# SyamVangara/multigrid-petsc

Hardware: AMD Instinct MI355X
Metric: fp64 DOF-updates/sec per V-cycle at 1024^3 (higher is better)
Workload: dtype f64

## Files before the change

include/mgk.h:

```cpp
#ifndef MGK_H
#define MGK_H
#include <stddef.h>
#ifdef __cplusplus
extern "C" {
#endif

#define MGK_XOFF 16
#define MGK_EINVAL  10001
#define MGK_ENOGPU  10002
#define MGK_ECOMM   10003

typedef struct mgk_ctx mgk_ctx;

typedef struct mgk_geom {
    int  dim;
    int  nx, ny, nz;
    int  pitch;
    long plane;
    long org;
    long total;
} mgk_geom;

int  mgk_geom_init(mgk_geom *g, int dim, int nx, int ny, int nz);

// ... 351 lines not shown
    MGK_TUNE_J2_RING_OLD       = 39,
    MGK_TUNE_SRR_TY2           = 40,
    MGK_TUNE_SRR_TY4           = 41,
    MGK_TUNE_J2_ZERO_RINGB     = 45,
    MGK_TUNE_PJ2_COPY          = 46,
    MGK_TUNE_J3_2D_MARCH       = 50,
    MGK_TUNE_J3_2D_CHUNK4      = 51,
    MGK_TUNE_J3_2D_CHUNK8      = 52,
    MGK_TUNE_DISPATCH_ORDER    = 53,
    MGK_TUNE_XCD_ORDER         = 54,
    MGK_TUNE_RR2D_MARCH        = 55,
    MGK_TUNE_RR2D_SHORT        = 56,
    MGK_TUNE_RESERVED_57       = 57,
    MGK_TUNE_J3_2D_ODD_DOWN    = 58,
    MGK_TUNE_J3_2D_ALL_DOWN    = 59,
    MGK_TUNE_J3_2D_STORE_PLAIN = 60,
    MGK_TUNE_J3_2D_STORE_NT    = 61,
    MGK_TUNE_J3_3D_TY2         = 62,
    MGK_TUNE_J3_3D_TY3         = 63,
    MGK_TUNE_J3_3D_ROWWISE     = 64,
    MGK_TUNE_NO_EXACT_FMA      = 65,
    MGK_TUNE_J3_3D_WAVES       = 66,
    MGK_TUNE_J3_3D_STACKED     = 67,
    MGK_TUNE_J3_3D_STACKED_DISPATCH = 68
};

void mgk_set_tuning(int variant, int zchunk);

#ifdef __cplusplus
}
#endif
#endif
```

include/mgk_sweep3.h:

```cpp
#ifndef MGK_SWEEP3_H
#define MGK_SWEEP3_H
#include "mgk.h"
#ifdef __cplusplus
extern "C" {
#endif

int  mgk_jacobi3_mid_ok_f64(const mgk_geom *g);
int  mgk_jacobi3_sumsq_mid_f64(mgk_ctx *ctx, const mgk_geom *g, const double *coef, double dinv, double scale,
                               const double *b, const double *u, double *unew, double *sumsq_host, void *stream);

#ifdef __cplusplus
}
#endif
#endif
```

include/mgsolve.h:

```cpp
#ifndef MGSOLVE_H
#define MGSOLVE_H
#include "mgk.h"
#ifdef __cplusplus
extern "C" {
#endif

typedef enum { MG_KSP_RICHARDSON = 0, MG_KSP_CHEBYSHEV = 1 } mg_ksp_type;
typedef enum { MG_PREC_FP64 = 0, MG_PREC_MIXED = 1 } mg_precision;
typedef enum { MG_PC_JACOBI = 0, MG_PC_LINE_Y = 1, MG_PC_LINE_X = 2, MG_PC_LINE_ALT = 3, MG_PC_RBGS = 4 } mg_pc_type;

typedef enum mg_fuse_bits {
    MG_FUSE_RESNORM = 1,
    MG_FUSE_PROLONG_SWEEP = 2,
    MG_FUSE_RES_RESTRICT = 4,
    MG_FUSE_NORM_SWEEP = 8,
    MG_FUSE_MIXED_CORRECT = 16,
    MG_FUSE_PAIRS = 32,
    MG_FUSE_RES_RESTRICT_SMALL = 128,
    MG_FUSE_COARSE_ZERO_SWEEP = 256,
    MG_FUSE_LDS_TAIL = 512,
    MG_FUSE_SWEEP_RESTRICT = 1024,
    MG_FUSE_ZERO_TRIPLE = 2048,
    MG_FUSE_PROLONG_PAIR = 4096,
    MG_FUSE_TRIPLE_2D = 8192,
// ... 39 lines not shown
struct mg_comm;

int  mg_solver_create(mg_solver **s, const mg_config *cfg, struct mg_comm *comm);
void mg_solver_destroy(mg_solver *s);
const char *mg_last_error(void);

int  mg_solver_set_rhs_problem(mg_solver *s);
int  mg_solver_set_rhs_host(mg_solver *s, const double *b_compact);
int  mg_solver_reset(mg_solver *s);
int  mg_solver_solve(mg_solver *s);
int  mg_solver_cycles(mg_solver *s, int ncycles);
int  mg_solver_fmg(mg_solver *s, int nu);
int  mg_solver_solve_fmg(mg_solver *s, int nu);
int  mg_solver_solve_gmres(mg_solver *s, int restart);
int  mg_solver_sync(mg_solver *s);

int    mg_solver_iterations(const mg_solver *s);
double mg_solver_bnorm(const mg_solver *s);
const double *mg_solver_rnorm(const mg_solver *s);
double mg_solver_solve_seconds(const mg_solver *s);

int  mg_solver_num_levels(const mg_solver *s);
int  mg_solver_tail_level(const mg_solver *s);
int  mg_solver_level_n(const mg_solver *s, int level);
int  mg_solver_level_local_planes(const mg_solver *s, int level, int *z0);
long mg_solver_local_unknowns(const mg_solver *s);
double mg_solver_dof_updates_per_cycle(const mg_solver *s);

int  mg_solver_get_solution(mg_solver *s, double *u_compact);
int  mg_solver_error_norms(mg_solver *s, double err[3]);

int  mg_solver_profile(mg_solver *s, int enable);
int  mg_solver_profile_read(mg_solver *s, double *total_ms, int *launches);
int  mg_solver_profile_read_kind(mg_solver *s, int kind, double *total_ms, int *launches);

void mg_get_ranges(int totaln, int procs, int *ranges);
int  mg_grid_n(int npts, int grid);
long mg_grid_to_global(int dim, int n, int k, int i, int j);
void mg_global_to_grid(int dim, int n, long idx, int *k, int *i, int *j);
int  mg_slab_range(int npts, int levels_dist, int level, int rank, int nranks, int *z0, int *z1);

#ifdef __cplusplus
}
#endif
#endif
```

multigrid_petsc_amd/csrc/mg_solver.c:

```c
#include "mgsolve.h"
#include "mg_comm.h"
#include "mg_solver_internal.h"
#include <math.h>
#include <stdio.h>
#include <stdlib.h>
#include <string.h>
#include <time.h>

#define MG_PI 3.14159265358979323846
static __thread char g_mgerr[512] = "ok";
const char *mg_last_error(void) { return g_mgerr; }
static int mgfail(int code, const char *what) {
    snprintf(g_mgerr, sizeof(g_mgerr), "%s (code %d; kernel layer: %s)", what, code, mgk_last_error());
    return code;
}

typedef struct mg_ops {
    int esz;
    int (*jacobi_range)(mgk_ctx *, const mgk_geom *, const double *, double, double, const void *, const void *, void *, int, int, void *);
    int (*jacobi_zero)(mgk_ctx *, const mgk_geom *, double, double, const void *, void *, void *);
    int (*residual)(mgk_ctx *, const mgk_geom *, const double *, const void *, const void *, void *, void *);
    int (*restrict_fw)(mgk_ctx *, const mgk_geom *, const mgk_geom *, const void *, void *, void *);
    int (*prolong_add)(mgk_ctx *, const mgk_geom *, const mgk_geom *, const void *, void *, void *);
    int (*prolong_jacobi)(mgk_ctx *, const mgk_geom *, const mgk_geom *, const double *, double, double, const void *, const void *, const void *, void *, void *);
// ... 935 lines not shown
    }
    F->u_ghost_ok = 0;
    return 0;
}

static int pjp_ok(const mg_solver *s, int P) {
    const mg_level *L = &s->L[0];
    const int need = MG_FUSE_PROLONG_PAIR | MG_FUSE_SWEEP_RESTRICT | MG_FUSE_PAIRS | MG_FUSE_NORM_SWEEP | MG_FUSE_PROLONG_SWEEP | MG_FUSE_RESNORM;
    if ((s->cfg.fuse & need) != need || P != 0 || s->cfg.dim != 3 || s->cfg.mesh || s->cfg.ksp_type != MG_KSP_RICHARDSON) return 0;
    if (s->cfg.v[0] != 3 || s->levels < 2 || s->lgraph == 1 || L->n < s->cfg.pair_min_n || s->last_cycle) return 0;
    if (L->distributed) {
        const mg_level *Lc = &s->L[1];
        const int hi = s->cfg.rank < s->cfg.nranks - 1;
        if (!(s->cfg.fuse & MG_FUSE_PROLONG_PAIR_SLAB) || !Lc->distributed || !L->f[0].far || !Lc->f[0].far || L->nz_min < 8 || Lc->nz_min < 4) return 0;
        return mgk_prolong_jacobi2_slab_ok_f64(&L->f[0].g, &Lc->f[0].g, hi) && mgk_jacobi2_sumsq_ok_f64(&L->f[0].g);
    }
    return mgk_prolong_jacobi2_ok_f64(&L->f[0].g, &s->L[1].f[0].g) && mgk_jacobi2_sumsq_ok_f64(&L->f[0].g);
}
static int triple_mid_ok(const mg_solver *s) {
    if (!(s->cfg.fuse & MG_FUSE_TRIPLE_MID) || !mg_triple_mid_pass || !mg_triple_mid_fits) return 0;
    if (s->cfg.nranks != 1 || s->L[0].distributed || s->cfg.v[0] != 3 || s->lgraph == 1) return 0;
    return srr_ok(s, 0, 0) && mg_triple_mid_fits(s);
}
static int finalize_iterate(mg_solver *s) {
    if (!s->iterate_behind) return 0;
    mg_level *L = &s->L[0];
    mg_fset *F = &L->f[0];
    if (L->distributed) {
        CHK(ensure_u_ghosts(s, 0, L));
        CHK(mgk_jacobi_range_f64(s->ctx, &F->g, L->coef, L->dinv, s->cfg.scale, (const double *)F->b, (const double *)F->u, (double *)F->tmp, 0, F->g.nz, NULL));
    } else
    CHK(mgk_jacobi_f64(s->ctx, &F->g, L->coef, L->dinv, s->cfg.scale, (const double *)F->b, (const double *)F->u, (double *)F->tmp, NULL));
    swap_ptr(&F->u, &F->tmp);
    mgi_u_rewritten(F);
    s->iterate_behind = 0; s->spec_valid = 0;
    return 0;
}

static int prolong_smooth(mg_solver *s, int P, int l) {
    mg_level *Lf = &s->L[l], *Lc = &s->L[l + 1];
    mg_fset *F = &Lf->f[P], *Cq = &Lc->f[P];
    const mg_ops *O = &OPS[P];
    const int v0 = s->cfg.v[0];
    if (!(s->cfg.fuse & MG_FUSE_PROLONG_SWEEP) || (s->cfg.ksp_type != MG_KSP_RICHARDSON && !j3_2d_ok(s, P, l, v0)) || v0 < 1) {
        CHK(prolong_from(s, P, l));
        return smooth(s, P, l, v0, 0);
// ... 31 lines not shown
        CHK(mgk_stream_wait(s->ctx, cs, ms));
        Cq->u_ghost_pending = 0; Cq->u_ghost_ok = 1;
        F->u_ghost_pending = 0; F->u_ghost_ok = 1; F->b_ghost_ok = 1;
        if (split) {
            if (lo) CHK(PJ2S(0, 4));
            if (hi) CHK(PJ2S(nz - 2, nz));
        } else CHK(PJ2S(0, nz));
#undef PJ2S
        swap_ptr(&F->u, &F->tmp);
        mgi_u_rewritten(F);
        s->sweep_owed = 1;
        return 0;
    }
    if (l == 0 && pjp_ok(s, P)) {
        void *t = triple_mid_ok(s) ? prof_begin_kind(s, 0, 1) : NULL;
        int rc2 = mgk_prolong_jacobi2_f64(s->ctx, &F->g, &Cq->g, Lf->coef, Lf->dinv, s->cfg.scale, (const double *)F->b, (const double *)Cq->u,
                                          (const double *)F->u, (double *)F->tmp, NULL);
        prof_end(s, t);
        CHK(rc2);
        swap_ptr(&F->u, &F->tmp);
        mgi_u_rewritten(F);
        s->sweep_owed = 1;
        return 0;
    }
    mgk_geom gc = Cq->g;
    const void *ucoarse = Cq->u;
    if (Lf->distributed && !Lc->distributed) {
        int c0 = s->zstart[s->cfg.rank], c1 = s->zstart[s->cfg.rank + 1];
        gc.nz = c1 - c0;
        ucoarse = (const char *)Cq->u + (size_t)O->esz * (size_t)c0 * (size_t)Cq->g.plane;
    } else if (Lc->distributed) {
        CHK(begin_u_ghosts(s, P, Lc));
    }
    if (Lf->distributed && s->cfg.overlap && Lf->nz_min >= 4 && s->cfg.dim == 3) {
        const int nz = F->g.nz;
        CHK(begin_u_ghosts(s, P, Lf));
        CHK(O->prolong_jacobi_range(s->ctx, &F->g, &gc, Lf->coef, Lf->dinv, s->cfg.scale, F->b, ucoarse, F->u, F->tmp, 2, nz - 1, NULL));
        if (Lc->distributed) CHK(ensure_u_ghosts(s, P, Lc));
        CHK(ensure_u_ghosts(s, P, Lf));
        CHK(O->prolong_jacobi_range(s->ctx, &F->g, &gc, Lf->coef, Lf->dinv, s->cfg.scale, F->b, ucoarse, F->u, F->tmp, 0, 2, NULL));
        CHK(O->prolong_jacobi_range(s->ctx, &F->g, &gc, Lf->coef, Lf->dinv, s->cfg.scale, F->b, ucoarse, F->u, F->tmp, nz - 1, nz, NULL));
    } else {
        if (Lf->distributed && Lc->distributed) CHK(ensure_u_ghosts(s, P, Lc));
        CHK(ensure_u_ghosts(s, P, Lf));
        if (s->cfg.mesh) CHK(mgk_prolong_jacobi_rowcoef_f64(s->ctx, &F->g, &gc, Lf->ctab, Lf->dtab, s->cfg.scale, (const double *)F->b,
                                                            (const double *)ucoarse, (const double *)F->u, (double *)F->tmp, NULL));
// ... 464 lines not shown
    if (!rc) rc = finalize_iterate(s);
    if (rc) return rc;
    double *ss = (double *)malloc(sizeof(double) * (size_t)(ncycles > 0 ? ncycles : 1));
    if (!ss) return mgfail(MGK_EINVAL, "mg_solver_cycles: out of host memory");
    rc = reduce_slots(s, s->d_norms, ncycles, ss);
    if (rc) { free(ss); return mgfail(rc, "mg_solver_cycles: reading the deferred norms"); }
    for (int q = 0; q < ncycles; q++) s->rnorm[it0 + 1 + q] = sqrt(ss[q]);
    if (ncycles > 0) s->rchk = s->rnorm[it0 + ncycles];
    free(ss);
    return 0;
}

int mg_solver_sync(mg_solver *s) {
    CHK(mgk_sync(s->ctx, NULL));
    if (s->comm && s->comm->check) { int rcc = s->comm->check(s->comm); if (rcc) return mgfail(rcc, mg_comm_last_error()); }
    return 0;
}
int mg_solver_iterations(const mg_solver *s) { return s->iter; }
double mg_solver_bnorm(const mg_solver *s) { return s->bnorm; }
const double *mg_solver_rnorm(const mg_solver *s) { return s->rnorm; }
double mg_solver_solve_seconds(const mg_solver *s) { return s->solve_seconds; }
int mg_solver_num_levels(const mg_solver *s) { return s->levels; }
int mg_solver_tail_level(const mg_solver *s) { return s ? s->ltail : 0; }
int mg_solver_level_n(const mg_solver *s, int l) { return (l >= 0 && l < s->levels) ? s->L[l].n : -1; }
int mg_solver_level_local_planes(const mg_solver *s, int l, int *z0) {
    if (l < 0 || l >= s->levels) return -1;
    if (z0) *z0 = s->L[l].z0;
    return s->L[l].nzl;
}
long mg_solver_local_unknowns(const mg_solver *s) {
    const mgk_geom *g = &s->L[0].f[0].g;
    return (long)g->nx * g->ny * g->nz;
}
double mg_solver_dof_updates_per_cycle(const mg_solver *s) {
    double tot = 0.0;
    for (int l = 0; l < s->levels; l++) {
        double N = pow((double)s->L[l].n, (double)s->cfg.dim);
        int sweeps = (l == s->levels - 1 && s->levels > 1) ? s->cfg.v[1] : 2 * s->cfg.v[0];
        if (s->levels == 1) sweeps = s->cfg.v[0];
        tot += sweeps * N;
    }
    return tot;
}

int mgi_fail(int code, const char *what) { return mgfail(code, what); }
int mgi_upload(mg_solver *s, const double *h, size_t n, double **d) { return upload(s, h, n, d); }
// ... 30 lines not shown
```

multigrid_petsc_amd/csrc/mg_solver_internal.h:

```cpp
#ifndef MG_SOLVER_INTERNAL_H
#define MG_SOLVER_INTERNAL_H
#include "mgsolve.h"
#include "mg_comm.h"
#include "mg_cheby_coefs.h"

#define MG_MAX_LEVELS 32
#define MG_MAX_TIMERS 4096

#define MG_FUSE_POINT_JACOBI_PASSES (MG_FUSE_PROLONG_SWEEP | MG_FUSE_NORM_SWEEP | MG_FUSE_PAIRS | MG_FUSE_COARSE_ZERO_SWEEP | MG_FUSE_LDS_TAIL | \
                                     MG_FUSE_SWEEP_RESTRICT | MG_FUSE_ZERO_TRIPLE | MG_FUSE_PROLONG_PAIR | MG_FUSE_TRIPLE_2D | \
                                     MG_FUSE_PROLONG_PAIR_SLAB | MG_FUSE_CHEBY | MG_FUSE_TRIPLE_MID)
#define MG_FUSE_NO_ROW_TABLE_FORM   (MG_FUSE_MIXED_CORRECT | MG_FUSE_RES_RESTRICT_SMALL)

typedef struct mg_fset {
    mgk_geom g;
    void *u, *b, *rv, *tmp;
    int guess_nonzero;
    int u_ghost_ok;
    int u_ghost_pending;
    int jz_ready;
    int last_sweep_pending;
    int b_ghost_ok;
    int pre_done;
    void *far;
// ... 24 lines not shown
    mgk_ctx *ctx;
    mg_comm *comm;
    int levels, ldist;
    mg_level L[MG_MAX_LEVELS];
    int *zstart;
    double *rnorm;
    int rnorm_cap;
    int iter;
    double bnorm, rchk;
    int started;
    int deferring;
    double *d_norms; int d_norms_cap;
    double *pin; int pin_cap;
    int spec_valid;
    int sweep_owed;
    int last_cycle;
    int iterate_behind;
    double solve_seconds;
    int lgraph;
    int ltail;
    void *coarse_graph[2];
    void *graph_u[2], *graph_tmp[2];
    int graph_rerecorded;
    int prof_on, prof_n;
    void *timers[MG_MAX_TIMERS];
    unsigned char timer_kind[MG_MAX_TIMERS];
    int prof_kind;
    int ntimers_created;
    void *gm_field[MGK_KRYLOV_MAX + 3];
    int gm_nfields, gm_restart;
    double *gm_hdev;
};

enum { MG_CHEBY_ZERO = 0, MG_CHEBY_PLAIN = 1, MG_CHEBY_PROLONG = 2, MG_CHEBY_NORM = 3 };
extern int mg_cheby_pass(mg_solver *s, int l, int kind, double *sumsq) __attribute__((weak));
extern int mg_cheby_tail(mg_solver *s) __attribute__((weak));

extern int mg_line_tables(mg_solver *s, int l, const double *ctab_host) __attribute__((weak));
extern int mg_line_smooth(mg_solver *s, int l, int maxit) __attribute__((weak));
extern int mg_xline_tables(mg_solver *s, int l, const double *ctab_host) __attribute__((weak));
extern int mg_xline_smooth(mg_solver *s, int l, int maxit) __attribute__((weak));
extern int mg_line_chunk_tables(mg_solver *s, int l, const double *ctab_host) __attribute__((weak));
extern int mg_line_chunk_smooth(mg_solver *s, int l, int maxit) __attribute__((weak));
extern int mg_xline_chunk_tables(mg_solver *s, int l, const double *ctab_host) __attribute__((weak));
extern int mg_xline_chunk_smooth(mg_solver *s, int l, int maxit) __attribute__((weak));
extern int mg_line_tail(mg_solver *s) __attribute__((weak));
extern int mg_rbgs_smooth(mg_solver *s, int l, int maxit) __attribute__((weak));
extern int mg_rbgs_prolong_smooth(mg_solver *s, int l, int maxit) __attribute__((weak));
extern int mg_triple_mid_fits(const mg_solver *s) __attribute__((weak));
extern int mg_triple_mid_pass(mg_solver *s, double *sumsq) __attribute__((weak));
long mg_xline_stride(int n, int uniform);
void mg_xline_factor(int n, int rows, const double *ctab, long gs, double *g);

int    mgi_fail(int code, const char *what);
#define CHK(call) do { int rc_ = (call); if (rc_) return mgi_fail(rc_, #call); } while (0)
int    mgi_upload(mg_solver *s, const double *h, size_t n, double **d);
double mgi_wall(void);
int    mgi_start(mg_solver *s);
int    mgi_smooth(mg_solver *s, int l, int maxit);
int    mgi_vcycle_rooted(mg_solver *s, int l);
int    mgi_vcycle_once(mg_solver *s);
int    mgi_iterate(mg_solver *s);
int    mgi_finalize(mg_solver *s);
int    mgi_apply_cycle(mg_solver *s);
#endif
```

multigrid_petsc_amd/csrc/mg_triple.c:

```c
#include "mg_solver_internal.h"
#include "mgk_sweep3.h"
#include <stddef.h>

int mg_triple_mid_fits(const mg_solver *s) {
    const mg_level *L = &s->L[0];
    return s->cfg.dim == 3 && !L->distributed && mgk_jacobi3_mid_ok_f64(&L->f[0].g);
}

int mg_triple_mid_pass(mg_solver *s, double *sumsq) {
    mg_level *L = &s->L[0];
    mg_fset *F = &L->f[0];
    CHK(mgk_jacobi3_sumsq_mid_f64(s->ctx, &F->g, L->coef, L->dinv, s->cfg.scale, (const double *)F->b, (const double *)F->u, (double *)F->tmp,
                                  sumsq, NULL));
    return 0;
}
```

multigrid_petsc_amd/csrc/mgk_sweep3.hip:

```cpp
#include "mgk_dev.hpp"
#include "mgk_sweep3.h"
#include <type_traits>

struct J3dArgs {
    const double *u, *b, *uc;
    double *out;
    int nx, ny, nxc, nyc;
    long rs, crs;
    int ntx, yc, nwaves, xcd, bous, plainst;
    double a0, a2, a3, a4, a6, dinv, scale;
    double ch[6];
    const double *ctab, *dtab;
    double *partials;
    double *rout;
};
template <bool PRO, bool ZG, bool NORM, bool TAB, int YC, bool CHEB = false>
__global__ void __launch_bounds__(256) k_jacobi3_2d(const J3dArgs a) {
    using VT = V16<double>;
    constexpr bool ZU = PRO && ZG, ZS = ZG && !PRO;
    const int lane = threadIdx.x & 63;
    int bid = blockIdx.x;
    if (a.xcd) bid = (bid & 7) * (gridDim.x >> 3) + (bid >> 3);
    const int wid = __builtin_amdgcn_readfirstlane(bid * 4 + (threadIdx.x >> 6));
    const int tx = wid % a.ntx, cy = wid / a.ntx;
// ... 472 lines not shown
static int jacobi3_3d(mgk_ctx *c, const mgk_geom *g, const double *coef, double dinv, double scale, const double *b, const double *u, double *unew,
                      void *stream, int *norm_parts) {
    if (!c || !g || g->dim != 3 || !coef || !b || !u || !unew || u == unew || b == unew) return fail(MGK_EINVAL, "mgk_jacobi3_f64: bad arguments (3-D)");
    J33Args a; memset(&a, 0, sizeof(a));
    a.u = u + g->org; a.b = b + g->org; a.out = unew + g->org;
    a.nx = g->nx; a.ny = g->ny; a.nz = g->nz; a.rs = g->pitch; a.ms = g->plane;
    set_coef7(a, coef);
    a.dinv = dinv; a.scale = scale;
    const int ty = (g_variant == MGK_TUNE_J3_3D_TY2) ? 2 : (g_variant == MGK_TUNE_J3_3D_TY3 || NORM) ? 3 : 4;
    if (ty == 2) return jacobi3_3d_launch<2, NORM>(c, a, g, coef, norm_parts, stream);
    if (ty == 3) return jacobi3_3d_launch<3, NORM>(c, a, g, coef, norm_parts, stream);
    if constexpr (!NORM) return jacobi3_3d_launch<4, NORM>(c, a, g, coef, norm_parts, stream);
    else return fail(MGK_EINVAL, "mgk_jacobi3_sumsq_f64: tile height not built");
}
struct J3sArgs {
    const double *u, *b;
    double *out;
    int nx, ny, nz;
    long rs, ms;
    int ntx, nty, ntz, zc, xcd;
    double a0, a1, a2, a3, a4, a5, a6, dinv, scale;
    double *partials;
};
#define J3S_WAVES 8
#define J3S_ROWS 4
template <int R, int NORM, bool EX>
__global__ void __launch_bounds__(64 * J3S_WAVES) k_jacobi3s(const J3sArgs a) {
    constexpr int NW = J3S_WAVES, Y = NW * R - 6;
    constexpr unsigned XROW = 1024, XBUF = 3 * NW * 2 * XROW;
    using VT = V16<double>;
    __shared__ __attribute__((aligned(16))) char xch[2 * XBUF];
    const int lane = threadIdx.x & 63;
    const int w = __builtin_amdgcn_readfirstlane((int)(threadIdx.x >> 6));
    int bid = blockIdx.x;
    if (a.xcd) bid = (bid & 7) * (gridDim.x >> 3) + (bid >> 3);
    const bool live = bid < a.ntx * a.nty * a.ntz;
    const int tile = live ? bid : 0;
    const int tx = tile % a.ntx, ty = (tile / a.ntx) % a.nty, tz = tile / (a.ntx * a.nty);
    const int z0 = tz * a.zc, z1 = min(z0 + a.zc, a.nz);
    const int t0 = z0 - 4, tend = live ? z1 : t0;
    const int yb = ty * Y, yw = yb - 3 + w * R;
    const int x0 = 2 * (tx * 60 + lane - 2);
    const bool xin = (x0 >= 0 && x0 < a.nx);
    const bool lastvec = (x0 + 2 > a.nx);
    const bool store = (lane >= 2 && lane <= 61 && xin);
    const unsigned lo = (unsigned)(8 * min(x0, a.nx + 1) + 32);
    const char *__restrict__ ub_ = reinterpret_cast<const char *>(a.u) - 32;
    const char *__restrict__ bb_ = reinterpret_cast<const char *>(a.b) - 32;
    char *__restrict__ ob_ = reinterpret_cast<char *>(a.out) - 32;
    long uro[R], bro[R];
    unsigned long long rowm[R], rown[R];
#pragma unroll
    for (int q = 0; q < R; q++) {
        const int y = yw + q;
// ... 40 lines not shown
        for (int q = 0; q < R; q++) { s_[q][0] = madd<EX>(s_[q][0], a.a2, lane_up<true>(C[q].v[1])); s_[q][1] = madd<EX>(s_[q][1], a.a2, C[q].v[0]); }
#pragma unroll
        for (int q = 0; q < R; q++) { s_[q][0] = s_[q][0] + a.a3 * C[q].v[0]; s_[q][1] = s_[q][1] + a.a3 * C[q].v[1]; }
#pragma unroll
        for (int q = 0; q < R; q++) { s_[q][0] = madd<EX>(s_[q][0], a.a4, C[q].v[1]); s_[q][1] = madd<EX>(s_[q][1], a.a4, lane_dn<true>(C[q].v[0])); }
#pragma unroll
        for (int q = 0; q < R; q++) { const VT &nv = (q == R - 1) ? hn : C[q < R - 1 ? q + 1 : R - 1]; s_[q][0] = madd<EX>(s_[q][0], a.a5, nv.v[0]); s_[q][1] = madd<EX>(s_[q][1], a.a5, nv.v[1]); }
#pragma unroll
        for (int q = 0; q < R; q++) { s_[q][0] = madd<EX>(s_[q][0], a.a6, UP[q].v[0]); s_[q][1] = madd<EX>(s_[q][1], a.a6, UP[q].v[1]); }
#pragma unroll
        for (int q = 0; q < R; q++) {
            const double r0 = BB[q].v[0] - s_[q][0], r1 = BB[q].v[1] - s_[q][1];
            const double zz0 = r0 * a.dinv, zz1 = r1 * a.dinv;
            const double v0 = C[q].v[0] + a.scale * zz0, v1 = C[q].v[1] + a.scale * zz1;
            const unsigned long long mu = decltype(maskrows)::value ? (rowm[q] & zm) : ~0ull;
            OUT[q].v[0] = andm(v0, Mx0 & mu); OUT[q].v[1] = andm(v1, Mx1 & mu);
            if constexpr (decltype(norm)::value) {
                const unsigned long long mn = rown[q] & nm;
                const double n0 = andm(r0, mn), n1 = andm(r1, Mx1 & mn);
                nacc += n0 * n0; nacc += n1 * n1;
            }
        }
    };
    using yes = std::true_type; using no = std::false_type;
    const VT Z = v16_zero<double>();
    VT U[3][R];
    VT P[3][R];
    VT Q[3][R];
    VT B[3][R];
    ldu(U[0], t0 + 1); ldu(U[1], t0 + 2); ldu(U[2], t0 + 3);
    ldb(B[2], t0 + 2);
#pragma unroll
    for (int k = 0; k < 3; k++)
#pragma unroll
        for (int q = 0; q < R; q++) { P[k][q] = Z; Q[k][q] = Z; if (k < 2) B[k][q] = Z; }
    xput(0, 0, U[1][0], U[1][R - 1]);
    __syncthreads();
    auto step = [&](auto phc, int t) {
        constexpr int PH = decltype(phc)::value, S0 = PH % 3, S1 = (PH + 1) % 3, S2 = (PH + 2) % 3;
        const unsigned rb = (unsigned)((t - t0) & 1) * XBUF, wb = XBUF - rb;
        const unsigned long long z2m = (t + 2 >= 0 && t + 2 < a.nz) ? ~0ull : 0ull, z1m = (t + 1 >= 0 && t + 1 < a.nz) ? ~0ull : 0ull;
        const unsigned long long z2own = (t + 2 >= z0 && t + 2 < z1) ? ~0ull : 0ull, z1own = (t + 1 >= z0 && t + 1 < z1) ? ~0ull : 0ull;
        VT hs, hn;
        xget(rb, 0, hs, hn);
        stage(P[S2], U[S0], hs, U[S1], hn, U[S2], B[S2], z2m, yes{}, std::integral_constant<bool, NORM == 1>{}, z2own);
        ldu(U[S0], t + 4);
        if (t >= z0 - 2) {
            xget(rb, 1, hs, hn);
            stage(Q[S2], P[S0], hs, P[S1], hn, P[S2], B[S1], z1m, yes{}, std::integral_constant<bool, NORM == 2>{}, z1own);
            if (t >= z0) {
                VT O[R];
                xget(rb, 2, hs, hn);
                stage(O, Q[S0], hs, Q[S1], hn, Q[S2], B[S0], ~0ull, no{}, no{}, 0ull);
                char *pz = ob_ + 8 * (long)t * a.ms;
#pragma unroll
                for (int q = 0; q < R; q++)
                    if (store && rown[q]) stv_stream(reinterpret_cast<double *>(pz + bro[q] + (size_t)lo), O[q]);
            }
        }
        ldb(B[S0], t + 3);
        xput(wb, 0, U[S2][0], U[S2][R - 1]);
        xput(wb, 1, P[S2][0], P[S2][R - 1]);
        xput(wb, 2, Q[S2][0], Q[S2][R - 1]);
        __syncthreads();
    };
    for (int t = t0; t < tend; t += 3) {
        step(std::integral_constant<int, 0>{}, t);
        if (t + 1 < tend) step(std::integral_constant<int, 1>{}, t + 1);
        if (t + 2 < tend) step(std::integral_constant<int, 2>{}, t + 2);
    }
    if (NORM) {
        const double sb = block_sum(store ? nacc : 0.0, reinterpret_cast<double *>(xch));
        if (threadIdx.x == 0) a.partials[blockIdx.x] = sb;
    }
}
static bool jacobi3s_shape_ok(const mgk_geom *g) { return g && g->dim == 3 && (g->nx + 1 == 512 || g->nx + 1 == 1024); }
static int jacobi3s_takes(const mgk_geom *g) {
    if (g_variant == MGK_TUNE_J3_3D_STACKED || g_variant == MGK_TUNE_J3_3D_STACKED_DISPATCH) return 1;
    if (g_variant == MGK_TUNE_J3_3D_WAVES || g_variant == MGK_TUNE_J3_3D_TY2 || g_variant == MGK_TUNE_J3_3D_TY3 || g_variant == MGK_TUNE_J3_3D_ROWWISE ||
        g_variant == MGK_TUNE_DISPATCH_ORDER) return 0;
    return jacobi3s_shape_ok(g) ? 1 : 0;
}
template <int NORM>
static int jacobi3s(mgk_ctx *c, const mgk_geom *g, const double *coef, double dinv, double scale, const double *b, const double *u, double *unew,
                    void *stream, int *norm_parts, const char *who) {
    static thread_local char msg[160];
    if (!c || !g || g->dim != 3 || !coef || !b || !u || !unew || u == unew || b == unew) {
        snprintf(msg, sizeof(msg), "%s: bad arguments (3-D; unew must not be u or b)", who);
        return fail(MGK_EINVAL, msg);
    }
    if (!jacobi3s_shape_ok(g)) {
        snprintf(msg, sizeof(msg), "%s: the stacked three-sweep pass is built for whole 3-D grids with rows of 512 or 1024 (nx = 511, 1023)", who);
        return fail(MGK_EINVAL, msg);
    }
    constexpr int R = (NORM == 1) ? 3 : J3S_ROWS, Y = J3S_WAVES * R - 6;
    J3sArgs a; memset(&a, 0, sizeof(a));
    a.u = u + g->org; a.b = b + g->org; a.out = unew + g->org;
    a.nx = g->nx; a.ny = g->ny; a.nz = g->nz; a.rs = g->pitch; a.ms = g->plane;
    set_coef7(a, coef);
    a.dinv = dinv; a.scale = scale;
    a.ntx = ((g->nx + 1) / 2 + 59) / 60;
    a.nty = (g->ny + Y - 1) / Y;
    const long per = (long)a.ntx * a.nty;
    long best = 1; double bestc = 0.0;
    for (long n = 1; n <= 16 && g->nz / n >= 8; n++) {
        const double cost = (double)((per * n + 255) / 256) * (double)((g->nz + n - 1) / n + 12);
        if (n == 1 || cost < bestc) { best = n; bestc = cost; }
    }
    const Chunks ch = cut_chunks_n(c, g->nz, best, { 8,  true,  false,  true,  0, 0});
    a.zc = ch.len; a.ntz = (int)ch.count;
    unsigned nblk = (unsigned)(per * a.ntz);
    a.xcd = (g_variant != MGK_TUNE_J3_3D_STACKED_DISPATCH && nblk >= 64) ? 1 : 0;
    if (a.xcd) nblk = (nblk + 7u) & ~7u;
    if (NORM) {
        if (!norm_parts || (long)nblk > c->max_partials) { snprintf(msg, sizeof(msg), "%s: more blocks than partial slots", who); return fail(MGK_EINVAL, msg); }
        a.partials = c->partials;
        *norm_parts = (int)nblk;
    }
    if (exact_fma7(coef)) hipLaunchKernelGGL((k_jacobi3s<R, NORM, true>), dim3(nblk), dim3(64 * J3S_WAVES), 0, S(c, stream), a);
    else hipLaunchKernelGGL((k_jacobi3s<R, NORM, false>), dim3(nblk), dim3(64 * J3S_WAVES), 0, S(c, stream), a);
    HIPCHK(hipGetLastError());
    return 0;
}
extern "C" int mgk_jacobi3_f64(mgk_ctx *c, const mgk_geom *g, const double *coef, double dinv, double scale,
                               const double *b, const double *u, double *unew, void *stream) {
    if (jacobi3s_takes(g)) return jacobi3s<0>(c, g, coef, dinv, scale, b, u, unew, stream, nullptr, "mgk_jacobi3_f64");
    return jacobi3_3d<false>(c, g, coef, dinv, scale, b, u, unew, stream, nullptr);
}
extern "C" int mgk_jacobi3_mid_ok_f64(const mgk_geom *g) { return jacobi3s_shape_ok(g) ? 1 : 0; }
extern "C" int mgk_jacobi3_sumsq_mid_f64(mgk_ctx *c, const mgk_geom *g, const double *coef, double dinv, double scale,
                                         const double *b, const double *u, double *unew, double *sumsq_host, void *stream) {
    if (!sumsq_host) return fail(MGK_EINVAL, "mgk_jacobi3_sumsq_mid_f64: bad arguments");
    int nparts = 0;
    int rc = jacobi3s<2>(c, g, coef, dinv, scale, b, u, unew, stream, &nparts, "mgk_jacobi3_sumsq_mid_f64");
    if (rc) return rc;
    return finish_to_host(c, nparts, 1, S(c, stream), sumsq_host);
}
extern "C" int mgk_jacobi3_sumsq_f64(mgk_ctx *c, const mgk_geom *g, const double *coef, double dinv, double scale,
                                     const double *b, const double *u, double *unew, double *sumsq_host, void *stream) {
    if (!sumsq_host) return fail(MGK_EINVAL, "mgk_jacobi3_sumsq_f64: bad arguments");
    int nparts = 0;
    int rc = jacobi3s_takes(g) ? jacobi3s<1>(c, g, coef, dinv, scale, b, u, unew, stream, &nparts, "mgk_jacobi3_sumsq_f64")
                               : jacobi3_3d<true>(c, g, coef, dinv, scale, b, u, unew, stream, &nparts);
    if (rc) return rc;
    return finish_to_host(c, nparts, 1, S(c, stream), sumsq_host);
// ... 109 lines not shown
```

multigrid_petsc_amd/mgk.py:

```python
import contextlib
import ctypes as C
import enum
import numpy as np
from ._lib import load_mgk

c_dp = C.POINTER(C.c_double)


class Geom(C.Structure):
    _fields_ = [("dim", C.c_int), ("nx", C.c_int), ("ny", C.c_int), ("nz", C.c_int),
                ("pitch", C.c_int), ("plane", C.c_long), ("org", C.c_long), ("total", C.c_long)]


class MgkError(RuntimeError):
    pass


class Tune(enum.IntEnum):
    DEFAULT = -1
    STORE_PLAIN = 0
    STORE_NT = 1
    LDS_TILE = 30
    ROW = 31
    ROW_PD2 = 32
# ... 7 lines not shown
    SRR_TY2 = 40
    SRR_TY4 = 41
    J2_ZERO_RINGB = 45
    PJ2_COPY = 46
    J3_2D_MARCH = 50
    J3_2D_CHUNK4 = 51
    J3_2D_CHUNK8 = 52
    DISPATCH_ORDER = 53
    XCD_ORDER = 54
    RR2D_MARCH = 55
    RR2D_SHORT = 56
    RESERVED_57 = 57
    J3_2D_ODD_DOWN = 58
    J3_2D_ALL_DOWN = 59
    J3_2D_STORE_PLAIN = 60
    J3_2D_STORE_NT = 61
    J3_3D_TY2 = 62
    J3_3D_TY3 = 63
    J3_3D_ROWWISE = 64
    NO_EXACT_FMA = 65
    J3_3D_WAVES = 66
    J3_3D_STACKED = 67
    J3_3D_STACKED_DISPATCH = 68


@contextlib.contextmanager
def tuning(variant=-1, zchunk=-1):
    L = load_mgk()
    L.mgk_set_tuning.restype, L.mgk_set_tuning.argtypes = None, [C.c_int, C.c_int]
    L.mgk_set_tuning(int(variant), int(zchunk))
    try:
        yield
    finally:
        L.mgk_set_tuning(-1, -1)


def _sigs(L):
    vp, i, d, sz = C.c_void_p, C.c_int, C.c_double, C.c_size_t
    G = C.POINTER(Geom)
    S = {
        "mgk_geom_init": (i, [G, i, i, i, i]),
        "mgk_device_count": (i, []),
        "mgk_set_device": (i, [i]),
        "mgk_ctx_create": (i, [C.POINTER(vp), i]),
        "mgk_ctx_destroy": (None, [vp]),
        "mgk_last_error": (C.c_char_p, []),
# ... 83 lines not shown
        "mgk_prolong_jacobi_range_f64": (i, [vp, G, G, c_dp, d, d, vp, vp, vp, vp, i, i, vp]),
        "mgk_prolong_jacobi_range_f32": (i, [vp, G, G, c_dp, d, d, vp, vp, vp, vp, i, i, vp]),
        "mgk_residual_restrict_range_f64": (i, [vp, G, G, c_dp, vp, vp, vp, i, i, vp]),
        "mgk_residual_restrict_range_f32": (i, [vp, G, G, c_dp, vp, vp, vp, i, i, vp]),
        "mgk_residual_restrict_slab_f64": (i, [vp, G, G, G, c_dp, vp, vp, vp, i, vp, i, i, vp]),
        "mgk_residual_restrict_slab_f32": (i, [vp, G, G, G, c_dp, vp, vp, vp, i, vp, i, i, vp]),
        "mgk_residual_restrict_2d_f64": (i, [vp, G, G, c_dp, vp, vp, vp, vp, d, d, vp]),
        "mgk_sweep_residual_restrict_f64": (i, [vp, G, G, c_dp, d, d, vp, vp, vp, vp, vp, d, d, vp]),
        "mgk_sweep_residual_restrict_ok_f64": (i, [G, G]),
        "mgk_jacobi2_sumsq_f64": (i, [vp, G, c_dp, d, d, vp, vp, vp, C.POINTER(d), vp]),
        "mgk_jacobi2_sumsq_ok_f64": (i, [G]),
        "mgk_jacobi2_sumsq_mid_f64": (i, [vp, G, c_dp, d, d, vp, vp, vp, C.POINTER(d), vp]),
        "mgk_prolong_jacobi2_ok_f64": (i, [G, G]),
        "mgk_prolong_jacobi2_f64": (i, [vp, G, G, c_dp, d, d, vp, vp, vp, vp, vp]),
        "mgk_jacobi2_zero_ok_f64": (i, [G]),
        "mgk_jacobi2_zero_ok_f32": (i, [G]),
        "mgk_jacobi2_zero_f64": (i, [vp, G, c_dp, d, d, vp, vp, vp]),
        "mgk_jacobi2_zero_f32": (i, [vp, G, c_dp, d, d, vp, vp, vp]),
        "mgk_jacobi2_2d_sumsq_f64": (i, [vp, G, c_dp, d, d, vp, vp, vp, C.POINTER(d), vp]),
        "mgk_jacobi3_f64": (i, [vp, G, c_dp, d, d, vp, vp, vp, vp]),
        "mgk_jacobi3_sumsq_f64": (i, [vp, G, c_dp, d, d, vp, vp, vp, C.POINTER(d), vp]),
        "mgk_jacobi3_sumsq_mid_f64": (i, [vp, G, c_dp, d, d, vp, vp, vp, C.POINTER(d), vp]),
        "mgk_jacobi3_mid_ok_f64": (i, [G]),
        "mgk_jacobi3_2d_f64": (i, [vp, G, c_dp, d, d, vp, vp, vp, vp, vp, vp]),
        "mgk_jacobi3_2d_sumsq_f64": (i, [vp, G, c_dp, d, d, vp, vp, vp, vp, vp, C.POINTER(d), vp]),
        "mgk_jacobi3_2d_zero_f64": (i, [vp, G, c_dp, d, d, vp, vp, vp, vp, vp]),
        "mgk_jacobi3_2d_sumsq_store_f64": (i, [vp, G, c_dp, d, d, vp, vp, vp, vp, vp, vp, C.POINTER(d), vp]),
        "mgk_prolong_jacobi3_2d_f64": (i, [vp, G, G, c_dp, d, d, vp, vp, vp, vp, vp, vp, vp]),
        "mgk_cheby3_2d_f64": (i, [vp, G, c_dp, d, c_dp, vp, vp, vp, vp, vp, vp]),
        "mgk_cheby3_2d_sumsq_f64": (i, [vp, G, c_dp, d, c_dp, vp, vp, vp, vp, vp, C.POINTER(d), vp]),
        "mgk_cheby3_2d_zero_f64": (i, [vp, G, c_dp, d, c_dp, vp, vp, vp, vp, vp]),
        "mgk_prolong_cheby3_2d_f64": (i, [vp, G, G, c_dp, d, c_dp, vp, vp, vp, vp, vp, vp, vp]),
        "mgk_tail_cycle_cheby_f64": (i, [vp, G, i, C.POINTER(i), c_dp, c_dp, C.POINTER(vp), C.POINTER(vp), d, d, i, i, vp, vp, vp]),
        "mgk_sweep_residual_restrict_2d_f64": (i, [vp, G, G, c_dp, d, d, vp, vp, vp, vp, vp, d, d, vp]),
        "mgk_jacobi2_sumsq_slab_f64": (i, [vp, G, G, c_dp, d, d, vp, vp, vp, vp, i, i, i, i, i, C.POINTER(i), vp]),
        "mgk_jacobi2_sumsq_mid_slab_f64": (i, [vp, G, G, c_dp, d, d, vp, vp, vp, vp, i, i, i, i, i, C.POINTER(i), vp]),
        "mgk_prolong_jacobi2_slab_ok_f64": (i, [G, G, i]),
        "mgk_prolong_jacobi2_slab_f64": (i, [vp, G, G, G, G, c_dp, d, d, vp, vp, vp, vp, vp, vp, i, i, i, i, vp]),
        "mgk_sweep_residual_restrict_slab_ok_f64": (i, [G, G]),
        "mgk_sweep_residual_restrict_slab_f64": (i, [vp, G, G, G, c_dp, d, d, vp, vp, vp, vp, vp, vp, i, i, vp, i, i, vp]),
        "mgk_ctx_set_chunk_planes": (i, [vp, i]),
        "mgk_residual_f64_to_f32_jz": (i, [vp, G, G, c_dp, vp, vp, vp, vp, d, d, C.POINTER(d), vp]),
        "mgk_correct_residual_f64_f32_jz": (i, [vp, G, G, c_dp, vp, vp, vp, vp, vp, vp, d, d, C.POINTER(d), vp]),
        "mgk_tail_cycle_f64": (i, [vp, G, i, C.POINTER(i), c_dp, c_dp, d, i, i, vp, vp, vp]),
        "mgk_tail_fmg_f64": (i, [vp, G, i, C.POINTER(i), c_dp, c_dp, d, i, i, i, vp, vp, vp]),
        "mgk_interp_jacobi2_ok_f64": (i, [G, G]),
# ... 150 lines not shown
```

multigrid_petsc_amd/solver.py:

```python
import ctypes as C
import enum

import numpy as np

from ._lib import load_mgpetsc


class MgConfig(C.Structure):
    _fields_ = [("dim", C.c_int), ("npts", C.c_int), ("levels", C.c_int), ("v", C.c_int * 2),
                ("maxiter", C.c_int), ("ksp_type", C.c_int), ("scale", C.c_double),
                ("emin", C.c_double), ("emax", C.c_double), ("rtol", C.c_double),
                ("device", C.c_int), ("precision", C.c_int), ("rank", C.c_int), ("nranks", C.c_int),
                ("dist_min_n", C.c_int), ("fuse", C.c_int), ("overlap", C.c_int), ("graph", C.c_int),
                ("pair_min_n", C.c_int), ("slab_chunk", C.c_int), ("mesh", C.c_int), ("pc_type", C.c_int),
                ("line_tail", C.c_int), ("xline_chunk", C.c_int), ("line_chunk", C.c_int)]


class MgError(RuntimeError):
    pass


class Fuse(enum.IntFlag):
    RESNORM = 1
    PROLONG_SWEEP = 2
# ... 32 lines not shown
    L.mg_solver_create.restype = i
    L.mg_solver_create.argtypes = [C.POINTER(vp), C.POINTER(MgConfig), vp]
    L.mg_solver_destroy.argtypes = [vp]
    L.mg_last_error.restype = C.c_char_p
    for f in ("mg_solver_set_rhs_problem", "mg_solver_reset", "mg_solver_solve", "mg_solver_sync"):
        getattr(L, f).restype = i
        getattr(L, f).argtypes = [vp]
    L.mg_solver_set_rhs_host.restype = i
    L.mg_solver_set_rhs_host.argtypes = [vp, vp]
    L.mg_solver_cycles.restype = i
    L.mg_solver_cycles.argtypes = [vp, i]
    L.mg_solver_iterations.restype = i
    L.mg_solver_iterations.argtypes = [vp]
    L.mg_solver_bnorm.restype = d
    L.mg_solver_bnorm.argtypes = [vp]
    L.mg_solver_rnorm.restype = C.POINTER(d)
    L.mg_solver_rnorm.argtypes = [vp]
    L.mg_solver_solve_seconds.restype = d
    L.mg_solver_solve_seconds.argtypes = [vp]
    L.mg_solver_num_levels.restype = i
    L.mg_solver_num_levels.argtypes = [vp]
    L.mg_solver_tail_level.restype = i
    L.mg_solver_tail_level.argtypes = [vp]
    L.mg_solver_level_n.restype = i
    L.mg_solver_level_n.argtypes = [vp, i]
    L.mg_solver_level_local_planes.restype = i
    L.mg_solver_level_local_planes.argtypes = [vp, i, C.POINTER(i)]
    L.mg_solver_local_unknowns.restype = C.c_long
    L.mg_solver_local_unknowns.argtypes = [vp]
    L.mg_solver_dof_updates_per_cycle.restype = d
    L.mg_solver_dof_updates_per_cycle.argtypes = [vp]
    L.mg_solver_get_solution.restype = i
    L.mg_solver_get_solution.argtypes = [vp, vp]
    L.mg_solver_error_norms.restype = i
    L.mg_solver_error_norms.argtypes = [vp, C.POINTER(d)]
    L.mg_solver_profile.restype = i
    L.mg_solver_profile.argtypes = [vp, i]
    L.mg_solver_profile_read.restype = i
    L.mg_solver_profile_read.argtypes = [vp, C.POINTER(d), C.POINTER(i)]
    L.mg_solver_profile_read_kind.restype = i
    L.mg_solver_profile_read_kind.argtypes = [vp, i, C.POINTER(d), C.POINTER(i)]
    L.mg_get_ranges.argtypes = [i, i, vp]
    L.mg_grid_n.restype = i
    L.mg_grid_n.argtypes = [i, i]
    L.mg_grid_to_global.restype = C.c_long
    L.mg_grid_to_global.argtypes = [i, i, i, i, i]
# ... 116 lines not shown
        return self.L.mg_solver_bnorm(self.h)

    @property
    def rnorm(self):
        p = self.L.mg_solver_rnorm(self.h)
        return np.array([p[q] for q in range(self.iterations + 1)])

    @property
    def solve_seconds(self):
        return self.L.mg_solver_solve_seconds(self.h)

    @property
    def local_unknowns(self):
        return self.L.mg_solver_local_unknowns(self.h)

    @property
    def dof_updates_per_cycle(self):
        return self.L.mg_solver_dof_updates_per_cycle(self.h)

    @property
    def tail_level(self):
        return self.L.mg_solver_tail_level(self.h)

    def level_n(self, l):
        return self.L.mg_solver_level_n(self.h, l)

    def level_planes(self, l):
        z0 = C.c_int()
        nz = self.L.mg_solver_level_local_planes(self.h, l, C.byref(z0))
        return z0.value, nz

    def solution(self):
        u = np.empty(self.local_unknowns)
        self._chk(self.L.mg_solver_get_solution(self.h, u.ctypes.data_as(C.c_void_p)))
        return u

    def error_norms(self):
        e = (C.c_double * 3)()
        self._chk(self.L.mg_solver_error_norms(self.h, e))
        return np.array(list(e))

    def profile(self, on=True):
        self._chk(self.L.mg_solver_profile(self.h, int(on)))

    def profile_read(self, kind=0):
        ms, n = C.c_double(), C.c_int()
# ... 3 lines not shown
```

Baseline: 409.5 billion.

## Fuse coarse-grid prolongation into the stacked three-sweep Jacobi kernel

Adds a prolongation variant of the stacked three-sweep 3-D Jacobi kernel. It reads coarse-grid values into an LDS ring buffer and adds the trilinear interpolation correction to the fine iterate as planes stream in, ahead of the three sweeps. The post-smoothing path uses this kernel when the triple-mid fuse bit is set, in place of a separate prolong-add plus sweeps. This removes one full read and write of the fine grid per level, at the cost of extra LDS, registers and per-plane correction arithmetic inside an already heavy kernel.

```diff
diff --git a/include/mgk.h b/include/mgk.h
--- a/include/mgk.h
+++ b/include/mgk.h
@@ -397,7 +397,8 @@
     MGK_TUNE_NO_EXACT_FMA      = 65,
     MGK_TUNE_J3_3D_WAVES       = 66,
     MGK_TUNE_J3_3D_STACKED     = 67,
-    MGK_TUNE_J3_3D_STACKED_DISPATCH = 68
+    MGK_TUNE_J3_3D_STACKED_DISPATCH = 68,
+    MGK_TUNE_NO_PROLONG_TRIPLE = 69
 };
 
 void mgk_set_tuning(int variant, int zchunk);
diff --git a/include/mgk_sweep3.h b/include/mgk_sweep3.h
--- a/include/mgk_sweep3.h
+++ b/include/mgk_sweep3.h
@@ -9,6 +9,10 @@
 int  mgk_jacobi3_sumsq_mid_f64(mgk_ctx *ctx, const mgk_geom *g, const double *coef, double dinv, double scale,
                                const double *b, const double *u, double *unew, double *sumsq_host, void *stream);
 
+int  mgk_prolong_jacobi3_ok_f64(const mgk_geom *gf, const mgk_geom *gc);
+int  mgk_prolong_jacobi3_f64(mgk_ctx *ctx, const mgk_geom *gf, const mgk_geom *gc, const double *coef, double dinv, double scale,
+                             const double *b, const double *uc, const double *u, double *unew, void *stream);
+
 #ifdef __cplusplus
 }
 #endif
diff --git a/include/mgsolve.h b/include/mgsolve.h
--- a/include/mgsolve.h
+++ b/include/mgsolve.h
@@ -85,6 +85,7 @@
 
 int  mg_solver_num_levels(const mg_solver *s);
 int  mg_solver_tail_level(const mg_solver *s);
+int  mg_solver_prolong_triple_launches(const mg_solver *s, int level);
 int  mg_solver_level_n(const mg_solver *s, int level);
 int  mg_solver_level_local_planes(const mg_solver *s, int level, int *z0);
 long mg_solver_local_unknowns(const mg_solver *s);
diff --git a/multigrid_petsc_amd/csrc/mg_solver.c b/multigrid_petsc_amd/csrc/mg_solver.c
--- a/multigrid_petsc_amd/csrc/mg_solver.c
+++ b/multigrid_petsc_amd/csrc/mg_solver.c
@@ -981,6 +981,13 @@
     if (s->cfg.nranks != 1 || s->L[0].distributed || s->cfg.v[0] != 3 || s->lgraph == 1) return 0;
     return srr_ok(s, 0, 0) && mg_triple_mid_fits(s);
 }
+static int prolong_triple_ok(const mg_solver *s, int P, int l) {
+    if (!(s->cfg.fuse & MG_FUSE_TRIPLE_MID) || !mg_triple_prolong_pass || !mg_triple_prolong_fits) return 0;
+    if (P != 0 || s->cfg.dim != 3 || s->cfg.mesh || s->cfg.ksp_type != MG_KSP_RICHARDSON || s->cfg.pc_type != MG_PC_JACOBI || s->cfg.v[0] < 3) return 0;
+    if (s->cfg.nranks != 1 || s->L[l].distributed || s->L[l + 1].distributed) return 0;
+    if (s->lgraph && l >= s->lgraph - 1) return 0;
+    return mg_triple_prolong_fits(s, l);
+}
 static int finalize_iterate(mg_solver *s) {
     if (!s->iterate_behind) return 0;
     mg_level *L = &s->L[0];
@@ -1058,6 +1065,12 @@
         mgi_u_rewritten(F);
         s->sweep_owed = 1;
         return 0;
+    }
+    if (prolong_triple_ok(s, P, l)) {
+        CHK(mg_triple_prolong_pass(s, l));
+        swap_ptr(&F->u, &F->tmp);
+        mgi_u_rewritten(F);
+        return v0 > 3 ? smooth(s, P, l, v0 - 3, 0) : 0;
     }
     mgk_geom gc = Cq->g;
     const void *ucoarse = Cq->u;
@@ -1568,6 +1581,7 @@
 double mg_solver_solve_seconds(const mg_solver *s) { return s->solve_seconds; }
 int mg_solver_num_levels(const mg_solver *s) { return s->levels; }
 int mg_solver_tail_level(const mg_solver *s) { return s ? s->ltail : 0; }
+int mg_solver_prolong_triple_launches(const mg_solver *s, int l) { return (s && l >= 0 && l < s->levels) ? s->prolong_triple_launches[l] : 0; }
 int mg_solver_level_n(const mg_solver *s, int l) { return (l >= 0 && l < s->levels) ? s->L[l].n : -1; }
 int mg_solver_level_local_planes(const mg_solver *s, int l, int *z0) {
     if (l < 0 || l >= s->levels) return -1;
diff --git a/multigrid_petsc_amd/csrc/mg_solver_internal.h b/multigrid_petsc_amd/csrc/mg_solver_internal.h
--- a/multigrid_petsc_amd/csrc/mg_solver_internal.h
+++ b/multigrid_petsc_amd/csrc/mg_solver_internal.h
@@ -70,6 +70,7 @@
     void *coarse_graph[2];
     void *graph_u[2], *graph_tmp[2];
     int graph_rerecorded;
+    int prolong_triple_launches[MG_MAX_LEVELS];
     int prof_on, prof_n;
     void *timers[MG_MAX_TIMERS];
     unsigned char timer_kind[MG_MAX_TIMERS];
@@ -97,6 +98,8 @@
 extern int mg_rbgs_prolong_smooth(mg_solver *s, int l, int maxit) __attribute__((weak));
 extern int mg_triple_mid_fits(const mg_solver *s) __attribute__((weak));
 extern int mg_triple_mid_pass(mg_solver *s, double *sumsq) __attribute__((weak));
+extern int mg_triple_prolong_fits(const mg_solver *s, int l) __attribute__((weak));
+extern int mg_triple_prolong_pass(mg_solver *s, int l) __attribute__((weak));
 long mg_xline_stride(int n, int uniform);
 void mg_xline_factor(int n, int rows, const double *ctab, long gs, double *g);
 
diff --git a/multigrid_petsc_amd/csrc/mg_triple.c b/multigrid_petsc_amd/csrc/mg_triple.c
--- a/multigrid_petsc_amd/csrc/mg_triple.c
+++ b/multigrid_petsc_amd/csrc/mg_triple.c
@@ -14,3 +14,18 @@
                                   sumsq, NULL));
     return 0;
 }
+
+int mg_triple_prolong_fits(const mg_solver *s, int l) {
+    if (s->cfg.dim != 3 || l < 0 || l + 1 >= s->levels) return 0;
+    const mg_level *Lf = &s->L[l], *Lc = &s->L[l + 1];
+    return !Lf->distributed && !Lc->distributed && mgk_prolong_jacobi3_ok_f64(&Lf->f[0].g, &Lc->f[0].g);
+}
+
+int mg_triple_prolong_pass(mg_solver *s, int l) {
+    mg_level *L = &s->L[l];
+    mg_fset *F = &L->f[0], *Cq = &s->L[l + 1].f[0];
+    CHK(mgk_prolong_jacobi3_f64(s->ctx, &F->g, &Cq->g, L->coef, L->dinv, s->cfg.scale, (const double *)F->b, (const double *)Cq->u,
+                                (const double *)F->u, (double *)F->tmp, NULL));
+    s->prolong_triple_launches[l]++;
+    return 0;
+}
diff --git a/multigrid_petsc_amd/csrc/mgk_sweep3.hip b/multigrid_petsc_amd/csrc/mgk_sweep3.hip
--- a/multigrid_petsc_amd/csrc/mgk_sweep3.hip
+++ b/multigrid_petsc_amd/csrc/mgk_sweep3.hip
@@ -518,14 +518,21 @@
     double a0, a1, a2, a3, a4, a5, a6, dinv, scale;
     double *partials;
 };
+struct J3spArgs : J3sArgs {
+    const double *uc;
+    int nxc, nyc, nzc;
+    long crs, cms;
+};
 #define J3S_WAVES 8
 #define J3S_ROWS 4
-template <int R, int NORM, bool EX>
-__global__ void __launch_bounds__(64 * J3S_WAVES) k_jacobi3s(const J3sArgs a) {
+template <int R, int NORM, bool EX, bool PRO = false>
+__global__ void __launch_bounds__(64 * J3S_WAVES) k_jacobi3s(const typename std::conditional<PRO, J3spArgs, J3sArgs>::type a) {
     constexpr int NW = J3S_WAVES, Y = NW * R - 6;
     constexpr unsigned XROW = 1024, XBUF = 3 * NW * 2 * XROW;
+    constexpr int NCR = 3, LC = 66;
     using VT = V16<double>;
     __shared__ __attribute__((aligned(16))) char xch[2 * XBUF];
+    __shared__ __attribute__((aligned(16))) double cbf[PRO ? 3 * NW * NCR * LC : 1];
     const int lane = threadIdx.x & 63;
     const int w = __builtin_amdgcn_readfirstlane((int)(threadIdx.x >> 6));
     int bid = blockIdx.x;
@@ -612,6 +619,56 @@
             }
         }
     };
+    const int ev = (R & 1) ? ((yw & 1) ^ 1) : 0;
+    const double *ucl = nullptr;
+    long cro[NCR] = {0, 0, 0};
+    double *cbw = cbf + (unsigned)w * (NCR * LC) + (unsigned)lane;
+    if constexpr (PRO) {
+        const int jb = (yw - 1) >> 1;
+        ucl = a.uc + min(max(tx * 60 + lane - 2, -1), a.nxc);
+#pragma unroll
+        for (int j = 0; j < NCR; j++) cro[j] = (long)min(max(jb + j, -1), a.nyc) * a.crs;
+    }
+    auto cslot = [](int k) -> unsigned { return (unsigned)(((k % 3) + 3) % 3) * (NW * NCR * LC); };
+    auto ldc = [&](double (&cl)[NCR], int k) {
+        if constexpr (PRO) {
+            const double *pk = ucl + (long)min(max(k, -1), a.nzc) * a.cms;
+#pragma unroll
+            for (int j = 0; j < NCR; j++) cl[j] = pk[cro[j]];
+        }
+    };
+    auto stc = [&](const double (&cl)[NCR], int k) {
+        double *p = cbw + cslot(k) + 1;
+#pragma unroll
+        for (int j = 0; j < NCR; j++) p[j * LC] = cl[j];
+    };
+    auto correct = [&](VT (&P_)[R], int z) {
+        const bool two = ((z & 1) == 0);
+        const int kl = (z - 1) >> 1;
+        const double *cA = cbw + cslot(kl), *cB = cbw + cslot(kl + 1);
+        const double wk = two ? 0.5 : 1.0;
+        const unsigned long long zm = (z >= 0 && z < a.nz) ? ~0ull : 0ull;
+#pragma unroll
+        for (int q = 0; q < R; q++) {
+            const bool tworows = (((ev + q) & 1) != 0);
+            const int j0 = (ev + q) >> 1;
+            const double wi = tworows ? 0.5 : 1.0;
+            const double wh = wk * (wi * 0.5), w1 = wk * (wi * 1.0);
+            double s0 = 0.0, s1 = 0.0;
+            {
+                const double c0 = cA[j0 * LC], c1 = cA[j0 * LC + 1];
+                s0 += wh * c0; s0 += wh * c1; s1 += w1 * c1;
+                if (tworows) { const double d0 = cA[(j0 + 1) * LC], d1 = cA[(j0 + 1) * LC + 1]; s0 += wh * d0; s0 += wh * d1; s1 += w1 * d1; }
+            }
+            if (two) {
+                const double c0 = cB[j0 * LC], c1 = cB[j0 * LC + 1];
+                s0 += wh * c0; s0 += wh * c1; s1 += w1 * c1;
+                if (tworows) { const double d0 = cB[(j0 + 1) * LC], d1 = cB[(j0 + 1) * LC + 1]; s0 += wh * d0; s0 += wh * d1; s1 += w1 * d1; }
+            }
+            const unsigned long long mu = rowm[q] & zm;
+            P_[q].v[0] = andm(P_[q].v[0] + s0, Mx0 & mu); P_[q].v[1] = andm(P_[q].v[1] + s1, Mx1 & mu);
+        }
+    };
     using yes = std::true_type; using no = std::false_type;
     const VT Z = v16_zero<double>();
     VT U[3][R];
@@ -624,11 +681,26 @@
     for (int k = 0; k < 3; k++)
 #pragma unroll
         for (int q = 0; q < R; q++) { P[k][q] = Z; Q[k][q] = Z; if (k < 2) B[k][q] = Z; }
+    if constexpr (PRO) {
+        const int m = t0 >> 1;
+        double c0[NCR], c1[NCR], c2[NCR];
+        ldc(c0, m); ldc(c1, m + 1); ldc(c2, m + 2);
+        for (int i = threadIdx.x; i < 3 * NW * NCR; i += 64 * NW) cbf[i * LC] = 0.0;
+        stc(c0, m); stc(c1, m + 1); stc(c2, m + 2);
+        __syncthreads();
+        correct(U[0], t0 + 1); correct(U[1], t0 + 2);
+    }
     xput(0, 0, U[1][0], U[1][R - 1]);
     __syncthreads();
     auto step = [&](auto phc, int t) {
         constexpr int PH = decltype(phc)::value, S0 = PH % 3, S1 = (PH + 1) % 3, S2 = (PH + 2) % 3;
         const unsigned rb = (unsigned)((t - t0) & 1) * XBUF, wb = XBUF - rb;
+        double cnew[NCR];
+        const bool newc = PRO && ((t & 1) == 0);
+        if constexpr (PRO) {
+            if (newc) ldc(cnew, (t + 4) >> 1);
+            correct(U[S2], t + 3);
+        }
         const unsigned long long z2m = (t + 2 >= 0 && t + 2 < a.nz) ? ~0ull : 0ull, z1m = (t + 1 >= 0 && t + 1 < a.nz) ? ~0ull : 0ull;
         const unsigned long long z2own = (t + 2 >= z0 && t + 2 < z1) ? ~0ull : 0ull, z1own = (t + 1 >= z0 && t + 1 < z1) ? ~0ull : 0ull;
         VT hs, hn;
@@ -652,6 +724,7 @@
         xput(wb, 0, U[S2][0], U[S2][R - 1]);
         xput(wb, 1, P[S2][0], P[S2][R - 1]);
         xput(wb, 2, Q[S2][0], Q[S2][R - 1]);
+        if constexpr (PRO) { if (newc) stc(cnew, (t + 4) >> 1); }
         __syncthreads();
     };
     for (int t = t0; t < tend; t += 3) {
@@ -671,20 +744,28 @@
         g_variant == MGK_TUNE_DISPATCH_ORDER) return 0;
     return jacobi3s_shape_ok(g) ? 1 : 0;
 }
-template <int NORM>
+template <int NORM, bool PRO = false>
 static int jacobi3s(mgk_ctx *c, const mgk_geom *g, const double *coef, double dinv, double scale, const double *b, const double *u, double *unew,
-                    void *stream, int *norm_parts, const char *who) {
-    static thread_local char msg[160];
+                    void *stream, int *norm_parts, const char *who, const mgk_geom *gc = nullptr, const double *uc = nullptr) {
+    static_assert(!PRO || NORM == 0, "the prolongation form forms no norm");
+    static thread_local char msg[200];
     if (!c || !g || g->dim != 3 || !coef || !b || !u || !unew || u == unew || b == unew) {
         snprintf(msg, sizeof(msg), "%s: bad arguments (3-D; unew must not be u or b)", who);
         return fail(MGK_EINVAL, msg);
     }
+    if (PRO && (!gc || !uc || uc == unew || gc->dim != 3 || g->nx != 2 * gc->nx + 1 || g->ny != 2 * gc->ny + 1 || g->nz != 2 * gc->nz + 1)) {
+        snprintf(msg, sizeof(msg), "%s: bad arguments (the fine grid must be 2 n + 1 points of the coarse one in every direction; unew must not be uc)", who);
+        return fail(MGK_EINVAL, msg);
+    }
     if (!jacobi3s_shape_ok(g)) {
         snprintf(msg, sizeof(msg), "%s: the stacked three-sweep pass is built for whole 3-D grids with rows of 512 or 1024 (nx = 511, 1023)", who);
         return fail(MGK_EINVAL, msg);
     }
     constexpr int R = (NORM == 1) ? 3 : J3S_ROWS, Y = J3S_WAVES * R - 6;
-    J3sArgs a; memset(&a, 0, sizeof(a));
+    typename std::conditional<PRO, J3spArgs, J3sArgs>::type a; memset(&a, 0, sizeof(a));
+    if constexpr (PRO) {
+        a.uc = uc + gc->org; a.nxc = gc->nx; a.nyc = gc->ny; a.nzc = gc->nz; a.crs = gc->pitch; a.cms = gc->plane;
+    }
     a.u = u + g->org; a.b = b + g->org; a.out = unew + g->org;
     a.nx = g->nx; a.ny = g->ny; a.nz = g->nz; a.rs = g->pitch; a.ms = g->plane;
     set_coef7(a, coef);
@@ -707,10 +788,19 @@
         a.partials = c->partials;
         *norm_parts = (int)nblk;
     }
-    if (exact_fma7(coef)) hipLaunchKernelGGL((k_jacobi3s<R, NORM, true>), dim3(nblk), dim3(64 * J3S_WAVES), 0, S(c, stream), a);
-    else hipLaunchKernelGGL((k_jacobi3s<R, NORM, false>), dim3(nblk), dim3(64 * J3S_WAVES), 0, S(c, stream), a);
+    if (exact_fma7(coef)) hipLaunchKernelGGL((k_jacobi3s<R, NORM, true, PRO>), dim3(nblk), dim3(64 * J3S_WAVES), 0, S(c, stream), a);
+    else hipLaunchKernelGGL((k_jacobi3s<R, NORM, false, PRO>), dim3(nblk), dim3(64 * J3S_WAVES), 0, S(c, stream), a);
     HIPCHK(hipGetLastError());
     return 0;
+}
+extern "C" int mgk_prolong_jacobi3_ok_f64(const mgk_geom *gf, const mgk_geom *gc) {
+    if (g_variant == MGK_TUNE_NO_PROLONG_TRIPLE) return 0;
+    if (!jacobi3s_shape_ok(gf) || !gc || gc->dim != 3) return 0;
+    return (gf->nx == 2 * gc->nx + 1 && gf->ny == 2 * gc->ny + 1 && gf->nz == 2 * gc->nz + 1) ? 1 : 0;
+}
+extern "C" int mgk_prolong_jacobi3_f64(mgk_ctx *c, const mgk_geom *gf, const mgk_geom *gc, const double *coef, double dinv, double scale,
+                                       const double *b, const double *uc, const double *u, double *unew, void *stream) {
+    return jacobi3s<0, true>(c, gf, coef, dinv, scale, b, u, unew, stream, nullptr, "mgk_prolong_jacobi3_f64", gc, uc);
 }
 extern "C" int mgk_jacobi3_f64(mgk_ctx *c, const mgk_geom *g, const double *coef, double dinv, double scale,
                                const double *b, const double *u, double *unew, void *stream) {
diff --git a/multigrid_petsc_amd/mgk.py b/multigrid_petsc_amd/mgk.py
--- a/multigrid_petsc_amd/mgk.py
+++ b/multigrid_petsc_amd/mgk.py
@@ -53,6 +53,7 @@
     J3_3D_WAVES = 66
     J3_3D_STACKED = 67
     J3_3D_STACKED_DISPATCH = 68
+    NO_PROLONG_TRIPLE = 69
 
 
 @contextlib.contextmanager
@@ -182,6 +183,8 @@
         "mgk_jacobi3_sumsq_f64": (i, [vp, G, c_dp, d, d, vp, vp, vp, C.POINTER(d), vp]),
         "mgk_jacobi3_sumsq_mid_f64": (i, [vp, G, c_dp, d, d, vp, vp, vp, C.POINTER(d), vp]),
         "mgk_jacobi3_mid_ok_f64": (i, [G]),
+        "mgk_prolong_jacobi3_ok_f64": (i, [G, G]),
+        "mgk_prolong_jacobi3_f64": (i, [vp, G, G, c_dp, d, d, vp, vp, vp, vp, vp]),
         "mgk_jacobi3_2d_f64": (i, [vp, G, c_dp, d, d, vp, vp, vp, vp, vp, vp]),
         "mgk_jacobi3_2d_sumsq_f64": (i, [vp, G, c_dp, d, d, vp, vp, vp, vp, vp, C.POINTER(d), vp]),
         "mgk_jacobi3_2d_zero_f64": (i, [vp, G, c_dp, d, d, vp, vp, vp, vp, vp]),
diff --git a/multigrid_petsc_amd/solver.py b/multigrid_petsc_amd/solver.py
--- a/multigrid_petsc_amd/solver.py
+++ b/multigrid_petsc_amd/solver.py
@@ -78,6 +78,8 @@
     L.mg_solver_num_levels.argtypes = [vp]
     L.mg_solver_tail_level.restype = i
     L.mg_solver_tail_level.argtypes = [vp]
+    L.mg_solver_prolong_triple_launches.restype = i
+    L.mg_solver_prolong_triple_launches.argtypes = [vp, i]
     L.mg_solver_level_n.restype = i
     L.mg_solver_level_n.argtypes = [vp, i]
     L.mg_solver_level_local_planes.restype = i
@@ -240,6 +242,9 @@
     def tail_level(self):
         return self.L.mg_solver_tail_level(self.h)
 
+    def prolong_triple_launches(self, l):
+        return self.L.mg_solver_prolong_triple_launches(self.h, l)
+
     def level_n(self, l):
         return self.L.mg_solver_level_n(self.h, l)
 
```

Result: faster. 419.5 billion, median of 6 (+2.4%).
